# mhaseebtariq/doppel-speller

Hardware: AMD Instinct MI355X
Metric: candidate-pairs scored/sec (Jaccard top-k + Levenshtein), 100k x 500k titles (higher is better)
Workload: dtype f32 accumulate / f64 finalise (Jaccard), u8 + f64 ratio (Levenshtein)

## Files before the change

### doppel-speller_amd/csrc/ds_common.h

```cpp
#pragma once

#include <hip/hip_runtime.h>

#include <cstdarg>
#include <cstdint>
#include <cstdio>
#include <cstring>
#include <string>
#include <vector>

#include "doppel_amd.h"

namespace ds {

constexpr int kWideTileRows = 28672, kNarrowTileRows = 12288;
constexpr int64_t kNarrowMaxTruth = 5000000;
constexpr int kDenseThreads = 1024;
constexpr int kMaxQueryColumns = 128;
constexpr int kSignatureBits = 128;
constexpr int kSignatureWords = kSignatureBits / 32;
constexpr int kRowRecordWords = 8;
constexpr int kControlWords = 32;

__host__ __device__ inline uint64_t mix64(uint64_t x)
// ... 64 lines not shown

struct ds_index {
    int device = 0;
    int64_t n_truth = 0, n_columns = 0, nnz = 0, n_tiles = 0, n_quads = 0;
    int tile_rows = 0;
    float sums_min = 0.f;
    ds::DeviceBuffer<uint32_t> col_ptr;
    ds::DeviceBuffer<uint16_t> postings;
    ds::DeviceBuffer<uint16_t> posting_sums;
    ds::DeviceBuffer<float> idf32;
    ds::DeviceBuffer<float> sums32;
    ds::DeviceBuffer<float> tile_sums_min;
    ds::DeviceBuffer<float> tile_sums_max;
    ds::DeviceBuffer<uint32_t> signature;
    ds::DeviceBuffer<int8_t> sig_column;
    ds::DeviceBuffer<unsigned char> row_start;
    ds::DeviceBuffer<unsigned char> row_cols;
    bool forward_wide_start = false, forward_wide_cols = false;
    bool rows_sorted = false;
    bool literal_only = false;
    ds::DeviceBuffer<unsigned char> kernel_args;
    ds::DeviceBuffer<int32_t> control;
    ds::DeviceBuffer<int32_t> status;
    ds::DeviceBuffer<int32_t> slow_list;
    ds::DeviceBuffer<int32_t> take_order;
    ds::DeviceBuffer<int32_t> order_bins;
    ds::DeviceBuffer<unsigned long long> phase;
    hipStream_t stream = nullptr;
    int compute_units = 256;
    hipEvent_t event_begin = nullptr, event_fast = nullptr, event_dense = nullptr;
    bool attributes_set = false;
    bool count_bytes = false;
    bool query_order = true;
    int64_t last_queries = 0;
    std::vector<unsigned char> last_args;
    int (*resolve_ties)(ds_index *, hipStream_t, const std::vector<int32_t> &) = nullptr;
    ds::DeviceBuffer<double> row_scratch;
};

struct ds_titles {
    int device = 0;
    int64_t n = 0, stride = 0;
    bool has_counts = false;
    ds::DeviceBuffer<uint8_t> enc;
    ds::DeviceBuffer<uint8_t> len;
    ds::DeviceBuffer<uint32_t> counts;
    ds::DeviceBuffer<unsigned char> records;
    uint32_t records_n_truth = 0;
    uint8_t records_space = 0;
    ds::DeviceBuffer<int32_t> unit_queue;
    size_t unit_queue_next = 0;
    bool records_enabled = true;
    ds::DeviceBuffer<int32_t> exact_slots;
    int exact_hash_bits = 64;
};
```

### doppel-speller_amd/csrc/ds_jaccard.hip

```cpp
#include "ds_common.h"

namespace ds {
namespace wide {
int launch(ds_index *index, const int64_t *d_q_rowptr, const int32_t *d_q_cols, const double *d_q_maxint, int64_t Q,
           int32_t k, int32_t *d_out_rows, hipStream_t stream);
int collect(ds_index *index, hipStream_t stream, int64_t stats[32]);
}
namespace narrow {
int launch(ds_index *index, const int64_t *d_q_rowptr, const int32_t *d_q_cols, const double *d_q_maxint, int64_t Q,
           int32_t k, int32_t *d_out_rows, hipStream_t stream);
}
}

typedef int (*ds_launch_function)(ds_index *, const int64_t *, const int32_t *, const double *, int64_t, int32_t, int32_t *,
                                  hipStream_t);

static ds_launch_function launch_for(const ds_index *index)
{
    return index != nullptr && index->tile_rows == ds::kNarrowTileRows ? ds::narrow::launch : ds::wide::launch;
}

extern "C" {

int ds_jaccard_topk_device(ds_index *index, const int64_t *d_q_rowptr, const int32_t *d_q_cols,
                           const double *d_q_maxint, int64_t Q, int32_t k, int32_t *d_out_rows, void *stream)
{
    return launch_for(index)(index, d_q_rowptr, d_q_cols, d_q_maxint, Q, k, d_out_rows, static_cast<hipStream_t>(stream));
}

int ds_jaccard_status(ds_index *index, void *stream, int32_t *status, int64_t Q)
{
    DS_REQUIRE(index != nullptr && status != nullptr, "ds_jaccard_status: null argument");
    DS_REQUIRE(Q == index->last_queries, "ds_jaccard_status: Q=%lld but the last call had %lld queries", (long long)Q,
               (long long)index->last_queries);
    if (Q == 0) return DS_OK;
    DS_HIP(hipSetDevice(index->device));
    DS_HIP(hipStreamSynchronize(static_cast<hipStream_t>(stream)));
    DS_HIP(hipMemcpy(status, index->status.ptr, static_cast<size_t>(Q) * sizeof(int32_t), hipMemcpyDeviceToHost));
    return DS_OK;
}

int ds_index_option(ds_index *index, const char *name, int64_t value)
{
    DS_REQUIRE(index != nullptr && name != nullptr, "ds_index_option: null argument");
    if (std::strcmp(name, "count_bytes") == 0) {
        index->count_bytes = value != 0;
        return DS_OK;
    }
    if (std::strcmp(name, "query_order") == 0) {
        index->query_order = value != 0;
        return DS_OK;
    }
    ds::set_error("ds_index_option: unknown option '%s'", name);
    return DS_E_ARG;
}

int ds_jaccard_sync(ds_index *index, void *stream, int64_t stats[32])
{
    return ds::wide::collect(index, static_cast<hipStream_t>(stream), stats);
}

int ds_jaccard_topk(ds_index *index, const int64_t *q_rowptr, const int32_t *q_cols, const double *q_maxint,
                    int64_t Q, int32_t k, int32_t *out_rows)
{
    DS_REQUIRE(index != nullptr, "ds_jaccard_topk: null index");
    DS_REQUIRE(Q >= 0, "ds_jaccard_topk: negative query count");
    if (Q == 0) return DS_OK;
    DS_REQUIRE(q_rowptr && q_maxint && out_rows, "ds_jaccard_topk: null pointer");
    DS_REQUIRE(q_rowptr[0] == 0, "ds_jaccard_topk: q_rowptr[0] must be 0");
    const int64_t q_nnz = q_rowptr[Q];
    DS_REQUIRE(q_nnz >= 0 && (q_nnz == 0 || q_cols), "ds_jaccard_topk: bad q_rowptr / q_cols");
    DS_HIP(hipSetDevice(index->device));
    ds::DeviceBuffer<int64_t> d_rowptr;
    ds::DeviceBuffer<int32_t> d_cols, d_out;
    ds::DeviceBuffer<double> d_maxint;
    int status = d_rowptr.upload(q_rowptr, static_cast<size_t>(Q + 1));
    if (status == DS_OK) status = d_cols.upload(q_cols, static_cast<size_t>(q_nnz > 0 ? q_nnz : 0));
    if (status == DS_OK && q_nnz == 0) status = d_cols.allocate(1);
    if (status == DS_OK) status = d_maxint.upload(q_maxint, static_cast<size_t>(Q));
    if (status == DS_OK) status = d_out.allocate(static_cast<size_t>(Q) * static_cast<size_t>(k > 0 ? k : 1));
    if (status != DS_OK) return status;
    status = launch_for(index)(index, d_rowptr.ptr, d_cols.ptr, d_maxint.ptr, Q, k, d_out.ptr, index->stream);
    if (status != DS_OK) return status;
    status = ds::wide::collect(index, index->stream, nullptr);
    DS_HIP(hipMemcpy(out_rows, d_out.ptr, static_cast<size_t>(Q) * k * sizeof(int32_t), hipMemcpyDeviceToHost));
// ... 5 lines not shown
```

### doppel-speller_amd/csrc/ds_jaccard_impl.inc

```
#include <cfloat>
#include <type_traits>
#include <cstdlib>

#include "ds_common.h"

namespace ds {
namespace DS_GEOMETRY_NAME {

constexpr int kTile = DS_TILE_ROWS;
constexpr uint32_t kPadWord = kTile / 2;
constexpr uint32_t kPadQuad = kPadWord * 0x10001u;
__device__ __forceinline__ uint32_t posting_row(uint32_t posting) { return ((posting & 0x7fffu) << 1) | (posting >> 15); }
constexpr int kThreads = DS_THREADS;
constexpr int kWorkgroupsPerCu = DS_WGS_PER_CU;
static_assert(kTile % 4096 == 0 && kTile < 65536, "tile rows: whole scan iterations, 15-bit word indexes");
static_assert(kThreads >= 256 && kThreads % 64 == 0, "the radix histogram is cleared by threads 0..255");
constexpr int kCandidates = DS_CANDIDATES;
constexpr int kSelectSlack = 128;
constexpr int kPtrTiles = DS_PTR_TILES;

struct JaccardArgs {
    const uint32_t *col_ptr;
    const uint16_t *postings;
    const uint16_t *posting_sums;
// ... 5 lines not shown
    const int8_t *sig_column;
    const void *row_start;
    const void *row_cols;
    int32_t forward_wide_start, forward_wide_cols;
    const int64_t *q_rowptr;
    const int32_t *q_cols;
    const double *q_maxint;
    int32_t *out_rows;
    int32_t *status;
    int32_t *control;
    int32_t *slow_list;
    const int32_t *take_order;
    unsigned long long *phase;
    int64_t n_truth;
    int64_t n_columns;
    int64_t n_queries;
    int32_t n_tiles;
    int32_t k;
    int32_t sparse_quads;
    int32_t literal_only;
    int32_t rows_sorted;
    int32_t select_min;
    int32_t select_growth;
    int64_t n_quads;
    int64_t nnz;
    float sums_min;
};

enum { kCtlQueue = 0, kCtlSlowCount = 1, kCtlErrors = 2, kCtlExact = 3, kCtlSelects = 4, kCtlSlowQueue = 5,
       kCtlSparseTiles = 6, kCtlDenseTiles = 7, kCtlSkippedColumns = 8, kCtlReason = 9 ,
       kCtlRedos = 15 ,
       kCtlRefines = 16, kCtlRawEntries = 17, kCtlSurvivors = 18, kCtlRawSparse = 19,
       kCtlBytes = 28  };

constexpr int kEpochTiles = DS_EPOCH_TILES;
static_assert(kEpochTiles >= 1 && kEpochTiles <= 256 && (kEpochTiles & (kEpochTiles - 1)) == 0, "epoch: a power of two, at most 256 tiles");
constexpr bool kEpochInBytes = static_cast<long long>(kTile + 2) * kEpochTiles > 65536;
constexpr int kEpochShift = kEpochInBytes ? 16 : 14;
static_assert(kEpochInBytes || kTile + 2 <= (1 << kEpochShift), "a local row (or a padding row, kTile + 1) and the epoch bits share 16 bits");
constexpr int kScoreWords = kTile / 2 + 16;
constexpr int kOffLo = kScoreWords * 4;
constexpr int kOffRow = kOffLo + kCandidates * 4;
constexpr int kOffRaw = kOffRow + kCandidates * 4;
constexpr int kOffRawTile = kOffRaw + (kThreads / 64) * 64 * 4;
constexpr int kOffCols = kOffRawTile + (kEpochInBytes ? (kThreads / 64) * 64 : 0);
constexpr int kOffIdf = kOffCols + kMaxQueryColumns * 4;
constexpr int kOffMass = kOffIdf + kMaxQueryColumns * 4;
constexpr int kOffBitIdf = kOffMass + kMaxQueryColumns * 4;
constexpr int kOffFixed = kOffBitIdf + kSignatureBits * 4;
constexpr int kOffRank = kOffFixed + kMaxQueryColumns * 4;
constexpr int kOffOrder = kOffRank + kMaxQueryColumns;
constexpr int kOffSigBit = kOffOrder + kMaxQueryColumns;
constexpr int kOffMassTable = kOffSigBit + kMaxQueryColumns;
constexpr int kOffPtr = kOffMassTable + 256 * 4;
constexpr int kOffHist = kOffMassTable;
constexpr int kOffQuadPrefix = kOffPtr + kMaxQueryColumns * (kPtrTiles + 1) * 4;
constexpr int kOffQuadBase = kOffQuadPrefix + kMaxQueryColumns * 4;
constexpr int kDirItems = 64, kDirColumns = 64;
constexpr int kOffDirEntry = kOffQuadBase + kMaxQueryColumns * 4;
constexpr int kOffDirMask = kOffDirEntry + 2 * kDirColumns * 8;
constexpr int kOffDirCount = kOffDirMask + 2 * kDirItems * 8;
constexpr int kOffCtrl = kOffDirCount + 2 * kDirItems;
constexpr int kFastLdsBytes = kOffCtrl + 192;
static_assert((kFastLdsBytes + 256) * kWorkgroupsPerCu <= 160 * 1024, "LDS budget of one CU exceeded");
constexpr int kExactRows = kCandidates * 24 + kMaxQueryColumns * 5 + kThreads * 2 <= kTile * 2 ? kCandidates : ((kTile * 2 - kMaxQueryColumns * 5 - kThreads * 2) / 24) & ~7;
constexpr int kExactValueOffset = kExactRows * 16;
constexpr int kExactSortedOffset = kExactValueOffset + kExactRows * 8;
constexpr int kExactCountOffset = kExactSortedOffset + kMaxQueryColumns * 5;
static_assert(kExactValueOffset % 8 == 0 && kExactCountOffset % 4 == 0 && kExactCountOffset + kThreads * 2 <= kTile * 2,
              "exact-stage scratch fits the tile");
static_assert(kMaxQueryColumns == 128, "two ballots cover the query's columns");
constexpr int kKeep = (kCandidates + kThreads - 1) / kThreads;
constexpr int kSelectTrigger = kCandidates - kSelectSlack;
constexpr int kWaves = kThreads / 64;
constexpr float kFixedOne = 65000.f;
constexpr int kProbeMaxK = kThreads / 4;
static_assert(2 * kThreads <= kCandidates - kSelectSlack, "two samples per thread fit the candidate buffer");

enum { kLQuery = 0, kLCount, kLOverflow, kLDigit, kLRemain, kLCoef, kLPre, kLCut, kLKth0, kLKth1, kLBad, kLItems,
       kLUnused12 , kLNonEssential, kLMass, kLSparse, kLSigMask , kLQuant = kLSigMask + 4 , kLEnd,
       kLStartTile = 29 ,
       kLFloor = 37 ,
       kLAhead = 38 ,
       kLTileMask = 32 , kLTileSkip = 36 ,
       kLStats = 24 ,
       kLBytes = 30  };
static_assert(kLEnd <= kLStats && kLStats + 5 <= kLBytes && kLBytes + 2 <= 32 && kLBytes % 2 == 0, "LDS control words");
static_assert(kLTileSkip < kLFloor && kLFloor < kLAhead && kLAhead + 2 <= 48, "LDS control words 32..47");

__device__ __forceinline__ int uniform(int v) { return __builtin_amdgcn_readfirstlane(v); }
__device__ __forceinline__ uint32_t uniform(uint32_t v) { return static_cast<uint32_t>(__builtin_amdgcn_readfirstlane(static_cast<int>(v))); }
__device__ __forceinline__ float uniform(float v) { return __int_as_float(__builtin_amdgcn_readfirstlane(__float_as_int(v))); }
__device__ __forceinline__ bool uniform(bool v) { return __builtin_amdgcn_readfirstlane(v ? 1 : 0) != 0; }

__device__ __forceinline__ float round_down_positive(double x)
// ... 201 lines not shown
#else
#define DS_STAMP(slot) do { } while (0)
#define DS_COUNT(slot, value) do { } while (0)
#endif

template <bool kCountBytes, bool kSecondSample>
__global__ __launch_bounds__(kThreads, kWorkgroupsPerCu * kThreads / 256) void ds_jaccard_topk_kernel(const void *arguments)
{
    const __attribute__((address_space(4))) JaccardArgs &a =
        *reinterpret_cast<const __attribute__((address_space(4))) JaccardArgs *>(reinterpret_cast<uintptr_t>(arguments));
#ifdef DS_DIAGNOSTICS
    unsigned long long stamp_ = a.phase != nullptr ? __builtin_amdgcn_s_memtime() : 0ull;
    __shared__ unsigned long long phase_lds[16];
    if (threadIdx.x < 16) phase_lds[threadIdx.x] = 0ull;
#endif
    extern __shared__ __align__(16) unsigned char lds[];
    uint32_t *cand_key = reinterpret_cast<uint32_t *>(lds + kOffLo);
    int32_t *cand_row = reinterpret_cast<int32_t *>(lds + kOffRow);
    int32_t *cols = reinterpret_cast<int32_t *>(lds + kOffCols);
    float *idf = reinterpret_cast<float *>(lds + kOffIdf);
    uint8_t *rank = reinterpret_cast<uint8_t *>(lds + kOffRank);
    uint8_t *order = reinterpret_cast<uint8_t *>(lds + kOffOrder);
    float *mass_upto = reinterpret_cast<float *>(lds + kOffMass);
    int8_t *sig_bit = reinterpret_cast<int8_t *>(lds + kOffSigBit);
    float *bit_idf = reinterpret_cast<float *>(lds + kOffBitIdf);
    uint32_t *fixed = reinterpret_cast<uint32_t *>(lds + kOffFixed);
    uint32_t *iscores = reinterpret_cast<uint32_t *>(lds);
    uint16_t *mass_low = reinterpret_cast<uint16_t *>(lds + kOffMassTable);
    uint16_t *mass_high = mass_low + 256;
    uint32_t *ptr_cache = reinterpret_cast<uint32_t *>(lds + kOffPtr);
    uint32_t *quad_prefix = reinterpret_cast<uint32_t *>(lds + kOffQuadPrefix);
    uint32_t *quad_base = reinterpret_cast<uint32_t *>(lds + kOffQuadBase);
    uint2 *dir_entry = reinterpret_cast<uint2 *>(lds + kOffDirEntry);
    uint32_t *dir_mask = reinterpret_cast<uint32_t *>(lds + kOffDirMask);
    uint8_t *dir_count = reinterpret_cast<uint8_t *>(lds + kOffDirCount);
    uint32_t *hist = reinterpret_cast<uint32_t *>(lds + kOffHist);
    const ControlWords ctrl{reinterpret_cast<int32_t *>(lds + kOffCtrl)};

    const int tid = threadIdx.x, lane = tid & 63;
    const int wave = uniform(tid >> 6);
    const int k = a.k;
    const int64_t ptr_stride = static_cast<int64_t>(a.n_tiles) + 1;
    typedef const unsigned long long __attribute__((address_space(1))) *GlobalQuads;
    auto load_quad = [](GlobalQuads base, uint32_t at) {
        const unsigned long long bits = base[at];
        return make_uint2(static_cast<uint32_t>(bits), static_cast<uint32_t>(bits >> 32));
    };
    auto own_registers = [](const void *pointer) {
        const uint64_t bits = reinterpret_cast<uint64_t>(pointer);
        const uint32_t lo = uniform(static_cast<uint32_t>(bits)), hi = uniform(static_cast<uint32_t>(bits >> 32));
        return reinterpret_cast<GlobalQuads>((static_cast<uint64_t>(hi) << 32) | lo);
    };
    const GlobalQuads quads = own_registers(a.postings), sums_quads = own_registers(a.posting_sums);
    typedef const float __attribute__((address_space(4))) *ConstantFloats;
    const ConstantFloats tile_sums_min = reinterpret_cast<ConstantFloats>(reinterpret_cast<uintptr_t>(a.tile_sums_min));
    const ConstantFloats tile_sums_max = reinterpret_cast<ConstantFloats>(reinterpret_cast<uintptr_t>(a.tile_sums_max));

    for (int i = tid * 4; i < kScoreWords; i += kThreads * 4)
        *reinterpret_cast<uint4 *>(&iscores[i]) = make_uint4(0u, 0u, 0u, 0u);
    if (tid < 5) ctrl[kLStats + tid] = 0;
    if (tid < 2) ctrl[kLBytes + tid] = 0;
    __syncthreads();
    unsigned long long *requested = reinterpret_cast<unsigned long long *>(lds + kOffCtrl + kLBytes * 4);
    uint32_t query_units = 0;
    auto count_units = [&](uint32_t units) { if constexpr (kCountBytes) query_units += units; };

    for (;;) {
        if (tid == 0) {
// ... 16 lines not shown
        bool slow = a.literal_only != 0 || n64 > kMaxQueryColumns || n64 < 0 || !(maxint > 0.0) || !(maxint < 1e30);
        int reason = slow ? 0 : -1;
        const int n = slow ? 0 : static_cast<int>(n64);
        if (tid < n) {
            const int32_t column = a.q_cols[qbase + tid];
            const bool bad = column < 0 || column >= a.n_columns;
            if (bad) ctrl[kLBad] = 1;
            cols[tid] = bad ? 0 : column;
            const float value = bad ? 0.f : a.idf32[column];
            const int bit = bad ? -1 : static_cast<int>(a.sig_column[column]);
            idf[tid] = value;
            sig_bit[tid] = static_cast<int8_t>(bit);
            if (bit >= 0) bit_idf[bit] = value;
        }
        if constexpr (kCountBytes) query_units = static_cast<uint32_t>(9 * n + 24 + 7) >> 3;
        if (a.rows_sorted && !slow) {
            int below = 0;
            const float own = static_cast<float>(maxint);
            for (int t = tid; t < a.n_tiles; t += kThreads) below += a.tile_sums_max[t] < own;
            for (int d = 32; d > 0; d >>= 1) below += __shfl_xor(below, d);
            if (lane == 0 && below) atomicAdd(ctrl.at(kLStartTile), below);
        }
        __syncthreads();
        if (uniform(static_cast<int>(ctrl[kLBad]))) {
            if (tid == 0) {
                a.status[q] = kQueryErrorArg;
                atomicAdd(&a.control[kCtlErrors], 1);
            }
            for (int j = tid; j < k; j += kThreads) a.out_rows[q * k + j] = -1;
            __syncthreads();
            continue;
        }
        if (tid >= 64 && tid < kMaxQueryColumns) quad_prefix[tid] = 0xffffffffu;
        if (tid < 4 * kDirItems) dir_mask[tid] = 0u;
        if (tid < n) {
            const float mine = idf[tid];
            int r = 0;
            double below = 0.0;
#pragma unroll 8
            for (int i = 0; i < n; ++i) {
                const float other = idf[i];
                const bool first = (other < mine) | ((other == mine) & (i <= tid));
                r += first & (i != tid);
                below += first ? static_cast<double>(other) : 0.0;
            }
            rank[tid] = static_cast<uint8_t>(r);
            order[r] = static_cast<uint8_t>(tid);
            mass_upto[r] = round_up_positive(below * (1.0 + 3.814697265625e-06));
        }

        const float maxint32 = static_cast<float>(maxint);
        __syncthreads();
        const float total_mass = uniform(n > 0 ? fmaxf(maxint32, mass_upto[n - 1]) : maxint32);
        if (!slow && n > 0 && uniform(maxint32 < mass_upto[n - 1] * 0.999f)) { slow = true; reason = 0; }
        const float to_fixed = uniform(kFixedOne / total_mass), from_fixed = uniform(total_mass * (1.f / kFixedOne));
        if (tid < kMaxQueryColumns) {
            uint32_t off = 0;
            if (tid < n) {
                const uint32_t f = max(1u, static_cast<uint32_t>(idf[tid] * to_fixed + 0.5f));
                fixed[tid] = f;
                const double unit = static_cast<double>(from_fixed);
                off = static_cast<uint32_t>(fabs(static_cast<double>(idf[tid]) - f * unit) / unit * 65536.0) + 1u;
            }
            const uint32_t total_off = wave_inclusive_scan(off, lane);
            if (lane == 63) atomicAdd(ctrl.at(kLQuant), static_cast<int32_t>(total_off));
        }
        auto error_margin = [&]() {
// ... 122 lines not shown
                for (int e = tid; e < n * (span + 1); e += kThreads) {
                    const int j = e / (span + 1), i = e - j * (span + 1);
                    ptr_cache[e] = (i < width && DS_OK_INDEX(2, static_cast<int64_t>(cols[j]) * ptr_stride + block_start + i,
                                                            a.n_columns * ptr_stride))
                                       ? a.col_ptr[static_cast<int64_t>(cols[j]) * ptr_stride + block_start + i]
                                       : 0u;
                }
                count_units(static_cast<uint32_t>(n * width + 1) >> 1);
                __syncthreads();
            }
            const int bt = b - block_start;
            bounds.mass = pending_mass;
            if (__builtin_expect(rebuild_mass_table, 0)) {
                rebuild_mass_table = false;
                tables_fresh = true;
                if (tid < 4) ctrl[kLTileMask + tid] = static_cast<int32_t>(ctrl[kLSigMask + tid]);
                if (tid == 4) ctrl[kLTileSkip] = non_essential;
                if (tid < 256) {
                    const uint32_t skipped16 = static_cast<uint32_t>(ctrl[kLSigMask]) & 0xffffu;
                    float lacks_low = 0.f, lacks_high = 0.f;
                    for (int g = 0; g < 8; ++g) {
                        if (((skipped16 >> g) & 1u) && !((tid >> g) & 1)) lacks_low += bit_idf[g];
                        if (((skipped16 >> (g + 8)) & 1u) && !((tid >> g) & 1)) lacks_high += bit_idf[g + 8];
                    }
                    const float full_units = bounds.mass * to_fixed_high + 2.5f;
                    const uint32_t full = static_cast<uint32_t>(full_units < 65535.f ? full_units : 65535.f);
                    const uint32_t low = static_cast<uint32_t>(lacks_low * (1.f - 3.814697265625e-06f) * to_fixed_low);
                    const uint32_t high = static_cast<uint32_t>(lacks_high * (1.f - 3.814697265625e-06f) * to_fixed_low);
                    mass_low[tid] = static_cast<uint16_t>(full - min(low, full));
                    mass_high[tid] = static_cast<uint16_t>(min(high, 65535u));
                }
            }
            const bool sparse = tight && sparse_mode;
            auto build_map = [&](int tile_bt, uint32_t copy, bool at_start, bool &directory) {
                uint32_t *const mask = dir_mask + copy * (2 * kDirItems);
                if (!at_start) {
                    mask[lane] = 0u;
                    mask[64 + lane] = 0u;
                }
                uint2 *const entry = dir_entry + copy * kDirColumns;
                uint8_t *const count = dir_count + copy * kDirItems;
                uint32_t quads_of[2] = {0u, 0u}, begin_of[2] = {0u, 0u};
#pragma unroll
                for (int h = 0; h < 2; ++h) {
                    const int j = lane + 64 * h;
                    if (j < n && rank[j] >= non_essential) {
                        begin_of[h] = ptr_cache[j * (span + 1) + tile_bt];
                        quads_of[h] = ptr_cache[j * (span + 1) + tile_bt + 1] - begin_of[h];
                    }
                }
                const uint32_t scan0 = wave_inclusive_scan(quads_of[0], lane);
                uint32_t total = static_cast<uint32_t>(__builtin_amdgcn_readlane(static_cast<int>(scan0), 63));
                const uint32_t before0 = scan0 - quads_of[0];
                uint32_t before1 = 0;
                const unsigned long long started0 = __ballot(quads_of[0] != 0u);
                unsigned long long started1 = 0ull;
                if (n > 64) {
                    const uint32_t scan1 = wave_inclusive_scan(quads_of[1], lane);
                    before1 = total + scan1 - quads_of[1];
                    total += static_cast<uint32_t>(__builtin_amdgcn_readlane(static_cast<int>(scan1), 63));
                    started1 = __ballot(quads_of[1] != 0u);
                }
                const int lists0 = __popcll(started0), lists = lists0 + __popcll(started1);
                directory = total <= static_cast<uint32_t>(kDirItems * 64) && lists <= kDirColumns;
                if (directory) {
                    const uint32_t below0 = __builtin_amdgcn_mbcnt_hi(static_cast<uint32_t>(started0 >> 32),
                                                                      __builtin_amdgcn_mbcnt_lo(static_cast<uint32_t>(started0), 0u));
                    if (quads_of[0] != 0u) {
                        entry[below0] = make_uint2(begin_of[0] - before0, fixed[lane]);
                        atomicOr(&mask[(before0 >> 6) * 2 + ((before0 >> 5) & 1u)], 1u << (before0 & 31u));
                    }
                    if (n > 64) {
                        const uint32_t below1 = lists0 + __builtin_amdgcn_mbcnt_hi(static_cast<uint32_t>(started1 >> 32),
                                                                                   __builtin_amdgcn_mbcnt_lo(static_cast<uint32_t>(started1), 0u));
                        if (quads_of[1] != 0u) {
                            entry[below1] = make_uint2(begin_of[1] - before1, fixed[lane + 64]);
                            atomicOr(&mask[(before1 >> 6) * 2 + ((before1 >> 5) & 1u)], 1u << (before1 & 31u));
                        }
                    }
                    const uint2 bits = *reinterpret_cast<const uint2 *>(&mask[2 * lane]);
                    const uint32_t starts = static_cast<uint32_t>(__popc(bits.x) + __popc(bits.y));
                    count[lane] = static_cast<uint8_t>(wave_inclusive_scan(starts, lane) - starts);
                } else if (at_start) {
                    quad_prefix[lane] = lane < n ? before0 : 0xffffffffu;
                    quad_base[lane] = begin_of[0] - before0;
                    if (n > 64) {
                        quad_prefix[lane + 64] = lane + 64 < n ? before1 : 0xffffffffu;
                        quad_base[lane + 64] = begin_of[1] - before1;
                    }
                }
                return total;
            };
            auto locate_in = [&](uint32_t copy, bool directory, uint32_t total, int at, uint32_t &first, uint32_t &value) {
                const uint32_t g = static_cast<uint32_t>(at) * 64u + lane;
                if (directory) {
                    const uint2 bits = *reinterpret_cast<const uint2 *>(&dir_mask[copy * (2 * kDirItems) + 2 * at]);
                    const uint32_t before = dir_count[copy * kDirItems + at];
                    const uint32_t below = __builtin_amdgcn_mbcnt_hi(bits.y, __builtin_amdgcn_mbcnt_lo(bits.x, 0u));
                    const uint32_t own = ((lane < 32 ? bits.x : bits.y) >> (lane & 31)) & 1u;
                    const uint2 entry = dir_entry[copy * kDirColumns + ((before + below + own - 1u) & (kDirColumns - 1))];
                    first = entry.x + g;
                    value = entry.y;
                } else {
                    uint32_t c = 0;
#pragma unroll
                    for (uint32_t bit = kMaxQueryColumns / 2; bit > 0; bit >>= 1) {
                        const uint32_t t = c + bit;
                        c = quad_prefix[t] <= g ? t : c;
                    }
                    first = quad_base[c] + g;
                    value = fixed[c];
                }
                return g < total;
            };
            auto request_round = [&](uint32_t copy, bool directory, uint32_t total, int items, int round, bool keep,
                                     bool count_sparse, uint2 (&q)[kRound], uint2 (&info)[kRound], uint32_t (&value)[kRound],
                                     bool (&alive)[kRound]) {
#pragma unroll
                for (int u = 0; u < kRound; ++u) {
                    const int at = wave + (round + u) * kWaves;
                    uint32_t first = 0;
                    value[u] = 0;
                    alive[u] = at < items && locate_in(copy, directory, total, at, first, value[u]) &&
                               DS_OK_INDEX(3, first, a.n_quads);
                    q[u] = alive[u] ? load_quad(quads, first) : make_uint2(kPadQuad, kPadQuad);
                    if (keep)
                        info[u] = alive[u] ? load_quad(sums_quads, first) : make_uint2(0u, 0u);
                    if constexpr (kCountBytes) {
                        const unsigned long long loaded = __ballot(alive[u]);
                        if (count_sparse && lane == 0)
                            atomicAdd(requested, static_cast<unsigned long long>(__popcll(loaded)) * (keep ? 16u : 8u));
                    }
                }
            };
            raw_tile_base = static_cast<int64_t>(epoch_start) * kTile;
            raw_epoch_bits = kEpochInBytes ? static_cast<uint32_t>(b - epoch_start)
                                           : static_cast<uint32_t>(b - epoch_start) << (kEpochShift & 15);
            const bool epoch_end = b >= epoch_last;
            const bool map_ahead = !epoch_end && b + 1 < block_end;
            const uint32_t tile_copy = dir_copy;
            if (!map_ahead) {
                uint32_t *const other = dir_mask + (tile_copy ^ 1u) * (2 * kDirItems);
                other[lane] = 0u;
                other[64 + lane] = 0u;
            }
            bool use_directory = false;
            uint32_t total_quads = 0;
            if (ahead) {
                const uint32_t built = uniform(static_cast<uint32_t>(ctrl[kLAhead + static_cast<int>(tile_copy)]));
                total_quads = built & 0x7fffffffu;
                use_directory = (built >> 31) != 0u;
#ifdef DS_BOUNDS_CHECK
                {
                    uint32_t mine = 0;
                    for (int j = lane; j < n; j += 64)
                        if (rank[j] >= non_essential) mine += ptr_cache[j * (span + 1) + bt + 1] - ptr_cache[j * (span + 1) + bt];
                    for (int d = 32; d > 0; d >>= 1) mine += __shfl_xor(mine, d);
                    if (mine != total_quads) record_violation(a.control, 11, static_cast<int64_t>(total_quads), static_cast<int64_t>(mine));
                }
#endif
            }
            if (!use_directory) total_quads = build_map(bt, tile_copy, true, use_directory);
            ahead = map_ahead;
            dir_copy ^= 1u;
            const int n_items = static_cast<int>((total_quads + 63u) >> 6);
            auto locate = [&](int at, uint32_t &first, uint32_t &value) {
                return locate_in(tile_copy, use_directory, total_quads, at, first, value);
            };
            if constexpr (kCountBytes) {
                if (!sparse) count_units(total_quads);
            }
            DS_STAMP(1);

            const int64_t tile_base = static_cast<int64_t>(b) * kTile;
            int count_at_step = sparse ? 0 : uniform(static_cast<int>(ctrl[kLCount]));
            Bounds here = bounds;
            auto passes = [&](float s, float sums_lower_bound, float row_mass) {
                return (s > 0.f) & (s + row_mass >= here.pre) &
                       (s + row_mass >= here.coef * (sums_lower_bound + here.maxint32));
            };
            auto consider4 = [&](const uint32_t (&fixed_score)[4], const uint32_t (&local)[4],
                                 const float (&sums_lower_bound)[4], const float (&row_mass)[4]) {
                bool pass[4];
#pragma unroll
                for (int e = 0; e < 4; ++e)
                    pass[e] = passes(static_cast<float>(fixed_score[e]) * from_fixed, sums_lower_bound[e], row_mass[e]);
                if (__ballot(pass[0] || pass[1] || pass[2] || pass[3]) == 0) return;
#pragma unroll
                for (int e = 0; e < 4; ++e) append_raw(pass[e], fixed_score[e], local[e]);
            };

            int kept_round = 0;
#pragma unroll
            for (int u = 0; u < kRound; ++u) live[u] = false;
            const int count_before = count_at_step;
            for (int round = 0; wave + round * kWaves < n_items; round += kRound) {
                const bool keep = sparse && wave + (round + kRound) * kWaves >= n_items;
                kept_round = round;
                request_round(tile_copy, use_directory, total_quads, n_items, round, keep, sparse, quad, quad_info, quad_value, live);
                if (map_ahead && round == 0 && wave == (b & (kWaves - 1))) {
                    bool directory;
                    const uint32_t total = build_map(bt + 1, tile_copy ^ 1u, false, directory);
                    if (lane == 0) {
                        ctrl[kLAhead + static_cast<int>(tile_copy ^ 1u)] = static_cast<int32_t>(total | (directory ? 0x80000000u : 0u));
                    }
                }
                if (sparse) DS_STAMP(10);
#pragma unroll
                for (int u = 0; u < kRound; ++u) {
                    if (!live[u]) continue;
                    const uint32_t shifted = quad_value[u] << ((quad[u].x >> 11) & 16u);
                    atomicAdd(&iscores[quad[u].x & 0x7fffu], shifted);
                    atomicAdd(&iscores[(quad[u].x >> 16) & 0x7fffu], shifted);
                    atomicAdd(&iscores[quad[u].y & 0x7fffu], shifted);
                    atomicAdd(&iscores[(quad[u].y >> 16) & 0x7fffu], shifted);
                }
            }
            if (map_ahead && wave >= n_items && wave == (b & (kWaves - 1))) {
                bool directory;
                const uint32_t total = build_map(bt + 1, tile_copy ^ 1u, false, directory);
                if (lane == 0) {
                    ctrl[kLAhead + static_cast<int>(tile_copy ^ 1u)] = static_cast<int32_t>(total | (directory ? 0x80000000u : 0u));
                }
            }
            if (sparse) DS_STAMP(15);
            __syncthreads();
            DS_STAMP(sparse ? 6 : 2);
            {
                const float gate = uniform(bounds.coef * (tile_min + maxint32) * (1.f - 3.814697265625e-06f));
                if (gate > here.pre) here.pre = gate;
            }

            if (sparse) {
                ++sparse_tiles;
                if (__builtin_expect(tables_fresh, 0)) {
                    tables_fresh = false;
                    mass_units_max = uniform(static_cast<uint32_t>(mass_low[255]));
                }
                const uint32_t gate_fixed = [&]() {
                    const float units = here.pre * to_fixed_low - 2.f;
                    const uint32_t gate = units > 0.f ? static_cast<uint32_t>(units) : 0u;
                    return max(gate, mass_units_max);
                }();
                auto collect = [&]() {
#pragma unroll
                    for (int u = 0; u < kRound; ++u) {
                        if (__ballot(live[u]) == 0) continue;
                        const uint32_t word[4] = {quad[u].x & 0x7fffu, (quad[u].x >> 16) & 0x7fffu, quad[u].y & 0x7fffu,
                                                  (quad[u].y >> 16) & 0x7fffu};
                        const uint32_t shift = (quad[u].x >> 11) & 16u;
                        const uint32_t info[4] = {quad_info[u].x & 0xffffu, quad_info[u].x >> 16, quad_info[u].y & 0xffffu,
                                                  quad_info[u].y >> 16};
                        uint32_t least[4];
// ... 34 lines not shown
                    }
                };
                collect();
                for (int round = 0; round < kept_round; round += kRound) {
#pragma unroll
                    for (int u = 0; u < kRound; ++u) {
                        const int at = wave + (round + u) * kWaves;
                        uint32_t first = 0, value = 0;
                        live[u] = at < n_items && locate(at, first, value) && DS_OK_INDEX(3, first, a.n_quads);
                        quad[u] = live[u] ? load_quad(quads, first) : make_uint2(kPadQuad, kPadQuad);
                        quad_info[u] = live[u] ? load_quad(sums_quads, first) : make_uint2(0u, 0u);
                        if constexpr (kCountBytes) {
                            const unsigned long long loaded = __ballot(live[u]);
                            if (lane == 0) atomicAdd(requested, static_cast<unsigned long long>(__popcll(loaded)) * 16u);
                        }
                    }
                    collect();
                }
                DS_STAMP(13);
                if (epoch_end) flush_raw();
                DS_STAMP(14);
                __syncthreads();
                DS_STAMP(7);
                if (__builtin_expect(uniform(static_cast<int>(ctrl[kLOverflow])) != 0, 0)) {
                    if (++sparse_retries > 5) { slow = true; reason = 2; break; }
                    wanted_in = uniform(static_cast<int>(ctrl[kLCount]));
                    floor_shift = min(sparse_retries - 1, 3);
                    __syncthreads();
                    if (tid == 0) {
                        ctrl[kLCount] = kCandidates;
                        ctrl[kLOverflow] = 0;
                        atomicAdd(&a.control[kCtlRedos], 1);
                    }
                    if (tid < 2 * kDirItems) dir_mask[dir_copy * (2 * kDirItems) + tid] = 0u;
                    ahead = false;
                    __syncthreads();
                    redo_tile = true;
                    raw_count = 0;
                } else {
                    if (epoch_end) sparse_retries = 0;
                    DS_COUNT(kCtlRawSparse, ctrl[kLCount] - count_before);
                    if (!epoch_end) {
                        ++b;
                        continue;
                    }
                }
            }

            const int64_t rows_left = a.n_truth - tile_base;
            const int limit = rows_left >= kTile ? kTile : static_cast<int>((rows_left + 7) & ~int64_t(7));
            int r0 = sparse ? limit : 0;
            if (!sparse) ++dense_tiles;
            bool select_now = sparse && (redo_tile || (epoch_end && uniform(static_cast<int>(ctrl[kLCount])) >= next_select));
            int retries = 0;
            bool probed = false;
            int32_t drop_lo = redo_tile ? static_cast<int32_t>(raw_tile_base) : 0;
            int32_t drop_hi = redo_tile ? static_cast<int32_t>(tile_base + kTile) : 0;
            bool force_pending = redo_tile;
            while (r0 < limit || select_now) {
                bool force_select = force_pending;
                force_pending = false;
                if (r0 < limit && !tight && !probed && k <= (kSecondSample ? 2 : 1) * kProbeMaxK && count_at_step == 0) {
                    probed = true;
                    const float tile_max = tile_sums_max[b];
                    uint32_t best_fixed = 0u;
                    [[maybe_unused]] int best_group = -1;
                    for (int idx = tid * 8; idx < limit; idx += kThreads * 8) {
// ... 1072 lines not shown
    args.sums32 = index->sums32.ptr;
    args.tile_sums_min = index->tile_sums_min.ptr;
    args.tile_sums_max = index->tile_sums_max.ptr;
    args.rows = reinterpret_cast<const uint4 *>(index->signature.ptr);
    args.sig_column = index->sig_column.ptr;
    args.row_start = index->row_start.ptr;
    args.row_cols = index->row_cols.ptr;
    args.forward_wide_start = index->forward_wide_start ? 1 : 0;
    args.forward_wide_cols = index->forward_wide_cols ? 1 : 0;
    args.nnz = index->nnz;
    args.q_rowptr = d_q_rowptr;
    args.q_cols = d_q_cols;
    args.q_maxint = d_q_maxint;
    args.out_rows = d_out_rows;
    args.status = index->status.ptr;
    args.control = index->control.ptr;
    args.slow_list = index->slow_list.ptr;
    args.take_order = nullptr;
    if (index->query_order) {
        const int blocks = static_cast<int>(std::min<int64_t>((Q + 4 * kOrderThreads - 1) / (4 * kOrderThreads), 256));
        const int64_t chunk = (Q + blocks - 1) / blocks;
        DS_HIP(hipMemsetAsync(index->order_bins.ptr, 0, 2 * kOrderStride * sizeof(int32_t), stream));
        hipLaunchKernelGGL(ds_query_order_count_kernel, dim3(blocks), dim3(kOrderThreads), 0, stream, d_q_rowptr, Q, chunk,
                           index->order_bins.ptr);
        DS_HIP(hipGetLastError());
        hipLaunchKernelGGL(ds_query_order_place_kernel, dim3(blocks), dim3(kOrderThreads), 0, stream, d_q_rowptr, Q, chunk,
                           index->order_bins.ptr, index->take_order.ptr);
        DS_HIP(hipGetLastError());
        args.take_order = index->take_order.ptr;
    }
    args.phase = nullptr;
#ifdef DS_DIAGNOSTICS
    if (const char *timers = getenv("DS_PHASE_TIMERS"); timers != nullptr && timers[0] == '1') {
        if (index->phase.count == 0 && index->phase.allocate(16) != DS_OK) return DS_E_HIP;
        DS_HIP(hipMemsetAsync(index->phase.ptr, 0, 16 * sizeof(unsigned long long), stream));
        args.phase = index->phase.ptr;
    }
#endif
    args.n_truth = index->n_truth;
    args.n_columns = index->n_columns;
    args.n_queries = Q;
    args.n_tiles = static_cast<int32_t>(index->n_tiles);
    args.k = k;
    args.sparse_quads = 4096;
    args.sums_min = index->sums_min;
    args.literal_only = index->literal_only ? 1 : 0;
    args.rows_sorted = index->rows_sorted ? 1 : 0;
    args.select_min = std::max(k, 16);
    args.select_growth = 3;
    args.n_quads = index->n_quads;

    const int grid = static_cast<int>(std::min<int64_t>(Q, int64_t(index->compute_units) * kWorkgroupsPerCu));
    DS_HIP(hipMemsetAsync(index->control.ptr, 0, kControlWords * sizeof(int32_t), stream));
    DS_HIP(hipEventRecord(index->event_begin, stream));
    if (k > kMaxSelectK) {
        args.take_order = nullptr;
        index->last_args.assign(reinterpret_cast<const unsigned char *>(&args), reinterpret_cast<const unsigned char *>(&args) + sizeof(args));
        index->resolve_ties = &resolve_ties;
        hipLaunchKernelGGL(ds_jaccard_mark_rowscan_kernel, dim3(static_cast<unsigned>((Q + 255) / 256)), dim3(256), 0, stream, args);
        DS_HIP(hipGetLastError());
        DS_HIP(hipEventRecord(index->event_fast, stream));
        DS_HIP(hipEventRecord(index->event_dense, stream));
        return DS_OK;
    }
    const bool second_sample = k > kProbeMaxK && k <= 2 * kProbeMaxK;
    auto kernel = index->count_bytes ? (second_sample ? ds_jaccard_topk_kernel<true, true> : ds_jaccard_topk_kernel<true, false>)
                                     : (second_sample ? ds_jaccard_topk_kernel<false, true> : ds_jaccard_topk_kernel<false, false>);
    static_assert(sizeof(JaccardArgs) <= 512, "ds_index::kernel_args");
    index->last_args.assign(reinterpret_cast<const unsigned char *>(&args), reinterpret_cast<const unsigned char *>(&args) + sizeof(args));
    index->resolve_ties = &resolve_ties;
    if (index->kernel_args.count == 0 && index->kernel_args.allocate(512) != DS_OK) return DS_E_HIP;
    DS_HIP(hipMemcpyAsync(index->kernel_args.ptr, &args, sizeof(args), hipMemcpyHostToDevice, stream));
    hipLaunchKernelGGL(kernel, dim3(grid), dim3(kThreads), kFastLdsBytes, stream, static_cast<const void *>(index->kernel_args.ptr));
    DS_HIP(hipGetLastError());
    DS_HIP(hipEventRecord(index->event_fast, stream));
    hipLaunchKernelGGL(ds_jaccard_repeats_kernel, dim3(static_cast<unsigned>((Q + 3) / 4)), dim3(256), 0, stream, args);
    DS_HIP(hipGetLastError());
    hipLaunchKernelGGL(ds_jaccard_dense_kernel, dim3(index->compute_units), dim3(kDenseThreads), kDenseLdsBytes, stream, args);
    DS_HIP(hipGetLastError());
    DS_HIP(hipEventRecord(index->event_dense, stream));
    return DS_OK;
}

int collect(ds_index *index, hipStream_t stream, int64_t stats[32])
{
    DS_REQUIRE(index != nullptr, "ds_jaccard_sync: null index");
    DS_HIP(hipSetDevice(index->device));
    int32_t control[kControlWords] = {0};
    DS_HIP(hipMemcpyAsync(control, index->control.ptr, sizeof(control), hipMemcpyDeviceToHost, stream));
    DS_HIP(hipStreamSynchronize(stream));
#ifdef DS_DIAGNOSTICS
    if (index->phase.ptr != nullptr && getenv("DS_PHASE_DUMP") != nullptr) {
        unsigned long long phase[16] = {0};
        DS_HIP(hipMemcpy(phase, index->phase.ptr, sizeof(phase), hipMemcpyDeviceToHost));
        fprintf(stderr, "phase cycles:");
        for (int i = 0; i < 16; ++i) fprintf(stderr, " %d=%llu", i, phase[i]);
        fprintf(stderr, "\n");
    }
#endif
    if (stats) {
        stats[0] = control[kCtlSlowCount];
        stats[1] = control[kCtlErrors];
        stats[2] = control[kCtlExact];
        stats[3] = control[kCtlSelects];
        for (int i = 4; i < 16; ++i) stats[i] = 0;
        if (index->phase.count) {
            unsigned long long phase[16];
            DS_HIP(hipMemcpy(phase, index->phase.ptr, sizeof(phase), hipMemcpyDeviceToHost));
            for (int i = 0; i < 8; ++i) stats[4 + i] = static_cast<int64_t>(phase[i]);
        }
        stats[12] = control[kCtlSparseTiles];
        stats[13] = control[kCtlDenseTiles];
        stats[14] = control[kCtlSkippedColumns];
        std::memcpy(&stats[15], &control[kCtlBytes], sizeof(int64_t));
        for (int i = 0; i < 6; ++i) stats[16 + i] = control[kCtlReason + i];
        stats[22] = control[kCtlRefines];
        stats[23] = control[kCtlRawEntries];
        stats[24] = control[kCtlSurvivors];
        stats[25] = control[kCtlRawSparse];
        float fast_ms = 0.f, dense_ms = 0.f;
        if (index->last_queries > 0 && hipEventElapsedTime(&fast_ms, index->event_begin, index->event_fast) == hipSuccess &&
            hipEventElapsedTime(&dense_ms, index->event_fast, index->event_dense) == hipSuccess) {
            stats[26] = static_cast<int64_t>(fast_ms * 1000.f);
            stats[27] = static_cast<int64_t>(dense_ms * 1000.f);
        } else {
            stats[26] = stats[27] = 0;
        }
        stats[28] = control[24];
        stats[29] = static_cast<int64_t>(static_cast<uint32_t>(control[25])) | (static_cast<int64_t>(control[26]) << 32);
// ... 42 lines not shown
```

Measured before the change: 67.23 million.

## Add larger start-tile quad directory to avoid binary search on first dense tile

Adds a larger directory (start bits plus per-item prefix counts) for the first dense tile, placed in the candidate key LDS area. This lets big start tiles use the O(1) directory lookup instead of falling back to a binary search over quad prefixes. The per-item counts now sit just below each map, and the prefix scan runs over several 64-item passes with a carry. The change also adds a max_workgroups option, plus diagnostic counters that only exist under DS_DIAGNOSTICS. The risks are aliasing with the candidate array (checked only under DS_BOUNDS_CHECK) and the extra scan passes at tile start.

```diff
diff --git a/doppel-speller_amd/csrc/ds_common.h b/doppel-speller_amd/csrc/ds_common.h
--- a/doppel-speller_amd/csrc/ds_common.h
+++ b/doppel-speller_amd/csrc/ds_common.h
@@ -120,6 +120,7 @@
     bool attributes_set = false;
     bool count_bytes = false;
     bool query_order = true;
+    int max_workgroups = 0;
     int64_t last_queries = 0;
     std::vector<unsigned char> last_args;
     int (*resolve_ties)(ds_index *, hipStream_t, const std::vector<int32_t> &) = nullptr;
diff --git a/doppel-speller_amd/csrc/ds_jaccard.hip b/doppel-speller_amd/csrc/ds_jaccard.hip
--- a/doppel-speller_amd/csrc/ds_jaccard.hip
+++ b/doppel-speller_amd/csrc/ds_jaccard.hip
@@ -51,6 +51,11 @@
         index->query_order = value != 0;
         return DS_OK;
     }
+    if (std::strcmp(name, "max_workgroups") == 0) {
+        DS_REQUIRE(value >= 0 && value <= 1 << 20, "ds_index_option: max_workgroups %lld out of range", (long long)value);
+        index->max_workgroups = static_cast<int>(value);
+        return DS_OK;
+    }
     ds::set_error("ds_index_option: unknown option '%s'", name);
     return DS_E_ARG;
 }
diff --git a/doppel-speller_amd/csrc/ds_jaccard_impl.inc b/doppel-speller_amd/csrc/ds_jaccard_impl.inc
--- a/doppel-speller_amd/csrc/ds_jaccard_impl.inc
+++ b/doppel-speller_amd/csrc/ds_jaccard_impl.inc
@@ -61,6 +61,9 @@
        kCtlRedos = 15 ,
        kCtlRefines = 16, kCtlRawEntries = 17, kCtlSurvivors = 18, kCtlRawSparse = 19,
        kCtlBytes = 28  };
+enum { kPhaseStartQuads = 16, kPhaseStartItems = 17, kPhaseDenseBeyondSmall = 18 ,
+       kPhaseDenseBeyondSmallFirst = 19 , kPhaseStartSearched = 20 , kPhaseStartItemsMax = 21, kPhaseStartHistogram = 22 ,
+       kPhaseWords = 32 };
 
 constexpr int kEpochTiles = DS_EPOCH_TILES;
 static_assert(kEpochTiles >= 1 && kEpochTiles <= 256 && (kEpochTiles & (kEpochTiles - 1)) == 0, "epoch: a power of two, at most 256 tiles");
@@ -86,10 +89,15 @@
 constexpr int kOffQuadPrefix = kOffPtr + kMaxQueryColumns * (kPtrTiles + 1) * 4;
 constexpr int kOffQuadBase = kOffQuadPrefix + kMaxQueryColumns * 4;
 constexpr int kDirItems = 64, kDirColumns = 64;
+constexpr int kStartDirItems = kCandidates * 4 / 9 >= 512 ? 512 : kCandidates * 4 / 9 >= 256 ? 256 : 128;
+static_assert(kStartDirItems * 8 + kStartDirItems <= kCandidates * 4, "start bits + counts of the start-tile directory fit the candidate key array");
+static_assert(kStartDirItems % 64 == 0 && kStartDirItems >= kDirItems && kStartDirItems <= kThreads, "whole scan passes; one thread zeroes one item's start bits");
 constexpr int kOffDirEntry = kOffQuadBase + kMaxQueryColumns * 4;
-constexpr int kOffDirMask = kOffDirEntry + 2 * kDirColumns * 8;
-constexpr int kOffDirCount = kOffDirMask + 2 * kDirItems * 8;
-constexpr int kOffCtrl = kOffDirCount + 2 * kDirItems;
+constexpr int kDirCopyBytes = kDirItems + kDirItems * 8;
+constexpr int kOffDirMap = kOffDirEntry + 2 * kDirColumns * 8 + kDirItems;
+constexpr int kOffStartDirMap = kOffLo + kStartDirItems;
+constexpr int kOffCtrl = kOffDirEntry + 2 * kDirColumns * 8 + 2 * kDirCopyBytes;
+static_assert(kOffDirMap % 8 == 0 && kDirCopyBytes % 8 == 0 && kOffStartDirMap % 8 == 0, "start-bit pairs are read as uint2");
 constexpr int kFastLdsBytes = kOffCtrl + 192;
 static_assert((kFastLdsBytes + 256) * kWorkgroupsPerCu <= 160 * 1024, "LDS budget of one CU exceeded");
 constexpr int kExactRows = kCandidates * 24 + kMaxQueryColumns * 5 + kThreads * 2 <= kTile * 2 ? kCandidates : ((kTile * 2 - kMaxQueryColumns * 5 - kThreads * 2) / 24) & ~7;
@@ -357,8 +365,8 @@
     uint32_t *quad_prefix = reinterpret_cast<uint32_t *>(lds + kOffQuadPrefix);
     uint32_t *quad_base = reinterpret_cast<uint32_t *>(lds + kOffQuadBase);
     uint2 *dir_entry = reinterpret_cast<uint2 *>(lds + kOffDirEntry);
-    uint32_t *dir_mask = reinterpret_cast<uint32_t *>(lds + kOffDirMask);
-    uint8_t *dir_count = reinterpret_cast<uint8_t *>(lds + kOffDirCount);
+    auto dir_bits = [&](uint32_t map) { return reinterpret_cast<uint32_t *>(lds + map); };
+    auto map_of = [](uint32_t copy) { return static_cast<uint32_t>(kOffDirMap) + copy * static_cast<uint32_t>(kDirCopyBytes); };
     uint32_t *hist = reinterpret_cast<uint32_t *>(lds + kOffHist);
     const ControlWords ctrl{reinterpret_cast<int32_t *>(lds + kOffCtrl)};
 
@@ -441,7 +449,8 @@
             continue;
         }
         if (tid >= 64 && tid < kMaxQueryColumns) quad_prefix[tid] = 0xffffffffu;
-        if (tid < 4 * kDirItems) dir_mask[tid] = 0u;
+        if (tid < 4 * kDirItems) dir_bits(map_of(static_cast<uint32_t>(tid) / (2 * kDirItems)))[tid % (2 * kDirItems)] = 0u;
+        if (tid < kStartDirItems) *reinterpret_cast<uint2 *>(lds + kOffStartDirMap + 8 * tid) = make_uint2(0u, 0u);
         if (tid < n) {
             const float mine = idf[tid];
             int r = 0;
@@ -630,14 +639,20 @@
                 }
             }
             const bool sparse = tight && sparse_mode;
-            auto build_map = [&](int tile_bt, uint32_t copy, bool at_start, bool &directory) {
-                uint32_t *const mask = dir_mask + copy * (2 * kDirItems);
+            auto build_map = [&](int tile_bt, uint32_t copy, bool at_start, uint32_t &map) {
+                const bool start_tile_map = at_start && dense_tiles == 0;
+                map = start_tile_map ? static_cast<uint32_t>(kOffStartDirMap) : map_of(copy);
+                const uint32_t capacity = start_tile_map ? kStartDirItems * 64u : kDirItems * 64u;
+#ifdef DS_BOUNDS_CHECK
+                if (start_tile_map && lane == 0 && ctrl[kLCount] != 0)
+                    record_violation(a.control, 12, static_cast<int64_t>(ctrl[kLCount]), 0);
+#endif
+                uint32_t *const mask = dir_bits(map);
                 if (!at_start) {
                     mask[lane] = 0u;
                     mask[64 + lane] = 0u;
                 }
                 uint2 *const entry = dir_entry + copy * kDirColumns;
-                uint8_t *const count = dir_count + copy * kDirItems;
                 uint32_t quads_of[2] = {0u, 0u}, begin_of[2] = {0u, 0u};
 #pragma unroll
                 for (int h = 0; h < 2; ++h) {
@@ -660,7 +675,7 @@
                     started1 = __ballot(quads_of[1] != 0u);
                 }
                 const int lists0 = __popcll(started0), lists = lists0 + __popcll(started1);
-                directory = total <= static_cast<uint32_t>(kDirItems * 64) && lists <= kDirColumns;
+                const bool directory = total <= capacity && lists <= kDirColumns;
                 if (directory) {
                     const uint32_t below0 = __builtin_amdgcn_mbcnt_hi(static_cast<uint32_t>(started0 >> 32),
                                                                       __builtin_amdgcn_mbcnt_lo(static_cast<uint32_t>(started0), 0u));
@@ -676,9 +691,16 @@
                             atomicOr(&mask[(before1 >> 6) * 2 + ((before1 >> 5) & 1u)], 1u << (before1 & 31u));
                         }
                     }
-                    const uint2 bits = *reinterpret_cast<const uint2 *>(&mask[2 * lane]);
-                    const uint32_t starts = static_cast<uint32_t>(__popc(bits.x) + __popc(bits.y));
-                    count[lane] = static_cast<uint8_t>(wave_inclusive_scan(starts, lane) - starts);
+                    const int passes = at_start ? static_cast<int>((total + 4095u) >> 12) : 1;
+                    uint32_t carried = 0u;
+                    for (int pass = 0; pass < passes; ++pass) {
+                        const uint32_t item = static_cast<uint32_t>(pass) * 64u + lane;
+                        const uint2 bits = *reinterpret_cast<const uint2 *>(&mask[2 * item]);
+                        const uint32_t starts = static_cast<uint32_t>(__popc(bits.x) + __popc(bits.y));
+                        const uint32_t scan = wave_inclusive_scan(starts, lane);
+                        lds[map - 1u - item] = static_cast<uint8_t>(carried + scan - starts);
+                        carried += static_cast<uint32_t>(__builtin_amdgcn_readlane(static_cast<int>(scan), 63));
+                    }
                 } else if (at_start) {
                     quad_prefix[lane] = lane < n ? before0 : 0xffffffffu;
                     quad_base[lane] = begin_of[0] - before0;
@@ -687,13 +709,14 @@
                         quad_base[lane + 64] = begin_of[1] - before1;
                     }
                 }
+                if (!directory) map = 0u;
                 return total;
             };
-            auto locate_in = [&](uint32_t copy, bool directory, uint32_t total, int at, uint32_t &first, uint32_t &value) {
+            auto locate_in = [&](uint32_t copy, uint32_t map, uint32_t total, int at, uint32_t &first, uint32_t &value) {
                 const uint32_t g = static_cast<uint32_t>(at) * 64u + lane;
-                if (directory) {
-                    const uint2 bits = *reinterpret_cast<const uint2 *>(&dir_mask[copy * (2 * kDirItems) + 2 * at]);
-                    const uint32_t before = dir_count[copy * kDirItems + at];
+                if (map != 0u) {
+                    const uint2 bits = *reinterpret_cast<const uint2 *>(lds + map + 8u * static_cast<uint32_t>(at));
+                    const uint32_t before = lds[map - 1u - static_cast<uint32_t>(at)];
                     const uint32_t below = __builtin_amdgcn_mbcnt_hi(bits.y, __builtin_amdgcn_mbcnt_lo(bits.x, 0u));
                     const uint32_t own = ((lane < 32 ? bits.x : bits.y) >> (lane & 31)) & 1u;
                     const uint2 entry = dir_entry[copy * kDirColumns + ((before + below + own - 1u) & (kDirColumns - 1))];
@@ -711,7 +734,7 @@
                 }
                 return g < total;
             };
-            auto request_round = [&](uint32_t copy, bool directory, uint32_t total, int items, int round, bool keep,
+            auto request_round = [&](uint32_t copy, uint32_t map, uint32_t total, int items, int round, bool keep,
                                      bool count_sparse, uint2 (&q)[kRound], uint2 (&info)[kRound], uint32_t (&value)[kRound],
                                      bool (&alive)[kRound]) {
 #pragma unroll
@@ -719,7 +742,7 @@
                     const int at = wave + (round + u) * kWaves;
                     uint32_t first = 0;
                     value[u] = 0;
-                    alive[u] = at < items && locate_in(copy, directory, total, at, first, value[u]) &&
+                    alive[u] = at < items && locate_in(copy, map, total, at, first, value[u]) &&
                                DS_OK_INDEX(3, first, a.n_quads);
                     q[u] = alive[u] ? load_quad(quads, first) : make_uint2(kPadQuad, kPadQuad);
                     if (keep)
@@ -738,16 +761,16 @@
             const bool map_ahead = !epoch_end && b + 1 < block_end;
             const uint32_t tile_copy = dir_copy;
             if (!map_ahead) {
-                uint32_t *const other = dir_mask + (tile_copy ^ 1u) * (2 * kDirItems);
+                uint32_t *const other = dir_bits(map_of(tile_copy ^ 1u));
                 other[lane] = 0u;
                 other[64 + lane] = 0u;
             }
-            bool use_directory = false;
             uint32_t total_quads = 0;
+            uint32_t tile_map = 0u;
             if (ahead) {
                 const uint32_t built = uniform(static_cast<uint32_t>(ctrl[kLAhead + static_cast<int>(tile_copy)]));
                 total_quads = built & 0x7fffffffu;
-                use_directory = (built >> 31) != 0u;
+                if ((built >> 31) != 0u) tile_map = map_of(tile_copy);
 #ifdef DS_BOUNDS_CHECK
                 {
                     uint32_t mine = 0;
@@ -758,16 +781,32 @@
                 }
 #endif
             }
-            if (!use_directory) total_quads = build_map(bt, tile_copy, true, use_directory);
+            if (tile_map == 0u) total_quads = build_map(bt, tile_copy, true, tile_map);
             ahead = map_ahead;
             dir_copy ^= 1u;
             const int n_items = static_cast<int>((total_quads + 63u) >> 6);
             auto locate = [&](int at, uint32_t &first, uint32_t &value) {
-                return locate_in(tile_copy, use_directory, total_quads, at, first, value);
+                return locate_in(tile_copy, tile_map, total_quads, at, first, value);
             };
             if constexpr (kCountBytes) {
                 if (!sparse) count_units(total_quads);
             }
+#ifdef DS_DIAGNOSTICS
+            if (a.phase != nullptr && tid == 0 && !sparse) {
+                const bool first = dense_tiles == 0, large = tile_map == static_cast<uint32_t>(kOffStartDirMap);
+                if (first) {
+                    atomicAdd(&a.phase[kPhaseStartQuads], static_cast<unsigned long long>(total_quads));
+                    atomicAdd(&a.phase[kPhaseStartItems], static_cast<unsigned long long>(n_items));
+                    atomicMax(&a.phase[kPhaseStartItemsMax], static_cast<unsigned long long>(n_items));
+                    atomicAdd(&a.phase[kPhaseStartHistogram + min(n_items >> 5, 9)], 1ull);
+                    if (tile_map == 0u) atomicAdd(&a.phase[kPhaseStartSearched], 1ull);
+                }
+                if (tile_map == 0u || (large && total_quads > static_cast<uint32_t>(kDirItems * 64))) {
+                    atomicAdd(&a.phase[kPhaseDenseBeyondSmall], 1ull);
+                    if (first) atomicAdd(&a.phase[kPhaseDenseBeyondSmallFirst], 1ull);
+                }
+            }
+#endif
             DS_STAMP(1);
 
             const int64_t tile_base = static_cast<int64_t>(b) * kTile;
@@ -795,10 +834,11 @@
             for (int round = 0; wave + round * kWaves < n_items; round += kRound) {
                 const bool keep = sparse && wave + (round + kRound) * kWaves >= n_items;
                 kept_round = round;
-                request_round(tile_copy, use_directory, total_quads, n_items, round, keep, sparse, quad, quad_info, quad_value, live);
+                request_round(tile_copy, tile_map, total_quads, n_items, round, keep, sparse, quad, quad_info, quad_value, live);
                 if (map_ahead && round == 0 && wave == (b & (kWaves - 1))) {
-                    bool directory;
-                    const uint32_t total = build_map(bt + 1, tile_copy ^ 1u, false, directory);
+                    uint32_t next_map;
+                    const uint32_t total = build_map(bt + 1, tile_copy ^ 1u, false, next_map);
+                    const bool directory = next_map != 0u;
                     if (lane == 0) {
                         ctrl[kLAhead + static_cast<int>(tile_copy ^ 1u)] = static_cast<int32_t>(total | (directory ? 0x80000000u : 0u));
                     }
@@ -815,8 +855,9 @@
                 }
             }
             if (map_ahead && wave >= n_items && wave == (b & (kWaves - 1))) {
-                bool directory;
-                const uint32_t total = build_map(bt + 1, tile_copy ^ 1u, false, directory);
+                uint32_t next_map;
+                const uint32_t total = build_map(bt + 1, tile_copy ^ 1u, false, next_map);
+                const bool directory = next_map != 0u;
                 if (lane == 0) {
                     ctrl[kLAhead + static_cast<int>(tile_copy ^ 1u)] = static_cast<int32_t>(total | (directory ? 0x80000000u : 0u));
                 }
@@ -917,7 +958,7 @@
                         ctrl[kLOverflow] = 0;
                         atomicAdd(&a.control[kCtlRedos], 1);
                     }
-                    if (tid < 2 * kDirItems) dir_mask[dir_copy * (2 * kDirItems) + tid] = 0u;
+                    if (tid < 2 * kDirItems) dir_bits(map_of(dir_copy))[tid] = 0u;
                     ahead = false;
                     __syncthreads();
                     redo_tile = true;
@@ -2056,8 +2097,8 @@
     args.phase = nullptr;
 #ifdef DS_DIAGNOSTICS
     if (const char *timers = getenv("DS_PHASE_TIMERS"); timers != nullptr && timers[0] == '1') {
-        if (index->phase.count == 0 && index->phase.allocate(16) != DS_OK) return DS_E_HIP;
-        DS_HIP(hipMemsetAsync(index->phase.ptr, 0, 16 * sizeof(unsigned long long), stream));
+        if (index->phase.count == 0 && index->phase.allocate(kPhaseWords) != DS_OK) return DS_E_HIP;
+        DS_HIP(hipMemsetAsync(index->phase.ptr, 0, kPhaseWords * sizeof(unsigned long long), stream));
         args.phase = index->phase.ptr;
     }
 #endif
@@ -2074,7 +2115,8 @@
     args.select_growth = 3;
     args.n_quads = index->n_quads;
 
-    const int grid = static_cast<int>(std::min<int64_t>(Q, int64_t(index->compute_units) * kWorkgroupsPerCu));
+    int grid = static_cast<int>(std::min<int64_t>(Q, int64_t(index->compute_units) * kWorkgroupsPerCu));
+    if (index->max_workgroups > 0) grid = std::min(grid, index->max_workgroups);
     DS_HIP(hipMemsetAsync(index->control.ptr, 0, kControlWords * sizeof(int32_t), stream));
     DS_HIP(hipEventRecord(index->event_begin, stream));
     if (k > kMaxSelectK) {
@@ -2115,10 +2157,15 @@
     DS_HIP(hipStreamSynchronize(stream));
 #ifdef DS_DIAGNOSTICS
     if (index->phase.ptr != nullptr && getenv("DS_PHASE_DUMP") != nullptr) {
-        unsigned long long phase[16] = {0};
+        unsigned long long phase[kPhaseWords] = {0};
         DS_HIP(hipMemcpy(phase, index->phase.ptr, sizeof(phase), hipMemcpyDeviceToHost));
         fprintf(stderr, "phase cycles:");
         for (int i = 0; i < 16; ++i) fprintf(stderr, " %d=%llu", i, phase[i]);
+        fprintf(stderr, "\n");
+        fprintf(stderr, "start tile: quads %llu items %llu max items %llu left to the binary search %llu; dense tiles beyond the small directory %llu, "
+                        "first tiles among them %llu; start tiles by items / 32:", phase[kPhaseStartQuads], phase[kPhaseStartItems],
+                phase[kPhaseStartItemsMax], phase[kPhaseStartSearched], phase[kPhaseDenseBeyondSmall], phase[kPhaseDenseBeyondSmallFirst]);
+        for (int i = 0; i < 10; ++i) fprintf(stderr, " %llu", phase[kPhaseStartHistogram + i]);
         fprintf(stderr, "\n");
     }
 #endif
```

New measurement: 67.63 million, median of 6. No clear change (+0.6%).
